# zju3dv/LoG

Hardware: NVIDIA H100
Metric: gaussians_per_s_fwd_bwd (higher is better)
Workload: dtype f32

## Files before the change

### include/log_b200_raster.h

```cpp
#ifndef LOG_B200_RASTER_H
#define LOG_B200_RASTER_H

#include <stdint.h>

#ifdef __cplusplus
extern "C" {
#endif

#define LGR_ABI_VERSION 24
#define LGR_TILE 16

#define LGR_FILTER_ADD 0
#define LGR_FILTER_MAX 1
#define LGR_FILTER_NONE 2

#define LGR_E_BADARG (-1)
#define LGR_E_CAPACITY (-2)
#define LGR_E_UNSUPPORTED (-3)

typedef struct lgr_view {
  int32_t image_height, image_width;
  float tanfovx, tanfovy;
  float scale_modifier;
  int32_t sh_degree;
// ... 15 lines not shown
  uint32_t* contrib_entry_d;
  int32_t* contrib_count_d;
  const int32_t* last_contrib_d;
  const int32_t* region_count_d;
  int64_t region_cap;
  int32_t num_regions;
  int32_t num_channels;
  int32_t log_depth;
  float* splat_ext_d;
  const float* cov3D_precomp_d;
  float* dcov3D_d;
  const float* viewmatrix_d;
  const float* projmatrix_d;
  const float* campos_d;
  const float* bg_d;
} lgr_view;

#define LGR_SPLAT_FLOATS 12
#define LGR_GRAD_FLOATS 12
#define LGR_TILE_SCRATCH_INTS 33
#define LGR_CONTRIB_MAX_LIST (1 << 24)
#define LGR_META_INTS 8

int lgr_abi_version(void);

int lgr_compute_radius(int64_t n, const float* means3D_d, const float* scales_d, const float* rotations_d,
                       const float* projmatrix_d, const float* viewmatrix_d, float focal_x, float focal_y,
                       float tan_fovx, float tan_fovy, float* radii_d, void* stream);

int lgr_mark_visible(int64_t n, const float* means3D_d, const float* viewmatrix_d, uint8_t* visible_d, void* stream);
// ... 207 lines not shown
```

### log_b200/_capi.py

```python
import ctypes
import os

from .build import LIB_PATH

_i32, _i64, _f32, _vp = ctypes.c_int32, ctypes.c_int64, ctypes.c_float, ctypes.c_void_p

LGR_FILTER_ADD, LGR_FILTER_MAX, LGR_FILTER_NONE = 0, 1, 2
LGR_SPLAT_FLOATS = 12
LGR_GRAD_FLOATS = 12
LGR_META_INTS = 8
LGR_TILE_SCRATCH_INTS = 33
LGR_ABI_VERSION = 24
LGR_CONTRIB_MAX_LIST = 1 << 24
LGR_STAGE_HEADER_FLOATS = 64
LGR_ROW_FLOATS = 20

EXPORTS = ('lgr_abi_version', 'lgr_sort_smem_capacity', 'lgr_compute_radius', 'lgr_forward_project',
           'lgr_forward_render', 'lgr_forward_render_device_sized', 'lgr_backward', 'lgr_grad_scatter_add', 'lgr_grad_scatter_add_staged', 'lgr_point_compact', 'lgr_sparse_adam', 'lgr_profile_enable', 'lgr_profile_collect',
           'lgr_profile_kernel_name', 'lgr_shard_send', 'lgr_shard_recv_bin', 'lgr_blend_backward', 'lgr_shard_return_rows',
           'lgr_shard_gather', 'lgr_shard_recv_bin_aux', 'lgr_shard_return_packed', 'lgr_shard_gather_packed', 'lgr_tree_traverse', 'lgr_mark_visible',
           'lgr_ssim_forward', 'lgr_ssim_backward', 'lgr_depth_loss_forward', 'lgr_depth_loss_backward', 'lgr_depth_vis',
           'lgr_counter_update', 'lgr_log_step', 'lgr_prepare_cull', 'lgr_prepare_select')
LGR_SHARD_MAX_RANKS = 32
LGR_PROFILE_KERNELS = 12


class LgrView(ctypes.Structure):
    _fields_ = [('image_height', _i32), ('image_width', _i32), ('tanfovx', _f32), ('tanfovy', _f32),
                ('scale_modifier', _f32), ('sh_degree', _i32), ('sh_coeffs', _i32), ('filter_mode', _i32),
                ('want_aux', _i32), ('tile_row_begin', _i32), ('tile_row_end', _i32),
                ('num_owners', _i32), ('raw_params', _i32), ('band_ids_d', _vp), ('band_blk_d', _vp), ('band_count_d', _vp), ('band_rows_d', _vp), ('band_dsplat_d', _vp), ('tile_rank_d', _vp), ('gather_index_d', _vp), ('pid_map_d', _vp), ('contrib_id_d', _vp), ('contrib_entry_d', _vp), ('contrib_count_d', _vp), ('last_contrib_d', _vp),
                ('region_count_d', _vp), ('region_cap', _i64), ('num_regions', _i32), ('num_channels', _i32), ('log_depth', _i32), ('splat_ext_d', _vp), ('cov3D_precomp_d', _vp), ('dcov3D_d', _vp),
                ('viewmatrix_d', _vp), ('projmatrix_d', _vp), ('campos_d', _vp), ('bg_d', _vp)]


class LgrShardLayout(ctypes.Structure):
    _fields_ = [('num_ranks', _i32), ('my_rank', _i32), ('cap', _i64), ('off_count', _i64), ('off_splat', _i64),
                ('off_radii', _i64), ('off_gid', _i64), ('off_dsplat', _i64), ('off_weight', _i64), ('off_pcount', _i64)]


class LgrTree(ctypes.Structure):
    _fields_ = [('num_points', _i64), ('num_nodes', _i64), ('max_child', _i32), ('max_level', _i32),
                ('node_index_d', _vp), ('tree_d', _vp)]


def tree_scratch_ints(num_points, slots):
    return 8 + 2 * num_points + slots + 2 * ((slots + 255) // 256) + 2 + (slots + 3) // 4

# ... 190 lines not shown
```

### log_b200/csrc/lgr_bin.cu

```cuda
#include "lgr_common.cuh"
#include "lgr_prof.cuh"

namespace lgr {

constexpr int SCAN_THREADS = 1024;
constexpr int SORT_CAP_SMALL_FWD = 4096;

__global__ void __launch_bounds__(SCAN_THREADS)
tile_scan_kernel(int ntiles, int32_t* __restrict__ tile_start ,
                 int32_t* __restrict__ cursor ,
                 int32_t* __restrict__ meta, int small_cap) {
  __shared__ int warp_sum[SCAN_THREADS / 32];
  __shared__ int carry_s, maxl_s, nbig_s;
  const int tid = threadIdx.x, lane = tid & 31, wid = tid >> 5;
  if (tid == 0) { carry_s = 0; maxl_s = 0; nbig_s = 0; }
  __syncthreads();
  int local_max = 0;
  for (int base = 0; base < ntiles; base += SCAN_THREADS) {
    const int i = base + tid;
    const int c = (i < ntiles) ? cursor[i * CSTRIDE] + cursor[i * CSTRIDE + 1] : 0;
    local_max = max(local_max, c);
    int x = c;
#pragma unroll
    for (int o = 1; o < 32; o <<= 1) { const int y = __shfl_up_sync(0xffffffffu, x, o); if (lane >= o) x += y; }
// ... 128 lines not shown
            float4* z = reinterpret_cast<float4*>(v.band_dsplat + (int64_t)id * LGR_GRAD_FLOATS);
            z[0] = z[1] = z[2] = make_float4(0.f, 0.f, 0.f, 0.f);
          }
          i = id;
        }
      }
      int rad = 0;
      float4 r0 = make_float4(0.f, 0.f, 0.f, 0.f), r1 = r0;
      float depth = 0.f;
      if (live) {
        rad = radii[i];
        r0 = ldg4(splat + i * LGR_SPLAT_FLOATS);
        r1 = ldg4(splat + i * LGR_SPLAT_FLOATS + 4);
        depth = __ldg(splat + i * LGR_SPLAT_FLOATS + 11);
        live = rad > 0;
      }
      if (live && v.num_owners == 0 && v.band_dsplat) {
        float4* z = reinterpret_cast<float4*>(v.band_dsplat + i * LGR_GRAD_FLOATS);
        z[0] = z[1] = z[2] = make_float4(0.f, 0.f, 0.f, 0.f);
      }
      int x0 = 0, y0 = 0, x1 = 0, y1 = 0;
      uint32_t key = 0;
      if (live) {
        live = r1.z > 0.f;
        if (live) {
          key = __float_as_uint(depth);
          tile_rect_tight(r0.x, r0.y, rad, r1.z, r1.w, v.gx, v.gy, v.row0, v.row1, x0, y0, x1, y1);
        }
      }
      const int w = x1 - x0, cnt = live ? w * (y1 - y0) : 0;
      const int mine = cnt <= 4 ? cnt : 0;
      int incl = mine;
#pragma unroll
      for (int o = 1; o < 32; o <<= 1) { const int y = __shfl_up_sync(0xffffffffu, incl, o); if (lane >= o) incl += y; }
// ... 445 lines not shown
  LGR_CHECK_LAUNCH();
  return 0;
}

constexpr int LONG_SORT_GRID = 132;

int launch_bin_and_sort(const View& v, int64_t n, int64_t num_inst, int max_len, int num_long, const float* splat,
                        const int32_t* radii, int32_t* tile_start, int32_t* cursor, uint32_t* inst_key,
                        uint32_t* inst_val, uint32_t* inst_tmp, int32_t* sorted_ids, int32_t* meta_dev, cudaStream_t st) {
  if (n == 0) return 0;
  if (meta_dev) {
    const int nt = v.gx * (v.row1 - v.row0);
    clamp_lists_kernel<<<(nt + 256) / 256, 256, 0, st>>>(nt, num_inst, tile_start, meta_dev);
    LGR_CHECK_LAUNCH();
  }
  if (num_inst == 0 && v.num_owners == 0 && v.band_dsplat == nullptr) return 0;
  if (num_inst > 0 && (!inst_tmp || !sorted_ids)) return LGR_E_BADARG;
  const int ntiles = v.gx * (v.row1 - v.row0);
  const int part_smem = part_smem_bytes(v.row1 - v.row0);
  if (part_smem > 160 * 1024) return LGR_E_UNSUPPORTED;
  {
    cudaError_t e = cudaFuncSetAttribute(bin_partition_kernel, cudaFuncAttributeMaxDynamicSharedMemorySize, part_smem);
    if (e != cudaSuccess) return (int)e;
  }
  const int rounds = (int)max((int64_t)1, min((int64_t)PART_ROUNDS, n / ((int64_t)BIN_THREADS * 132 * 16)));
  const int64_t chunk = (int64_t)rounds * BIN_THREADS;
  unsigned blocks = (unsigned)((n + chunk - 1) / chunk);
  if (v.region_count && blocks > (unsigned)LGR_REGION_GRID) blocks = (unsigned)LGR_REGION_GRID;
  unsigned long long* stage = reinterpret_cast<unsigned long long*>(inst_tmp);
  {
    ProfScope ps(K_BIN_SCATTER, st, num_inst > BIN_DIRECT_MAX ? 2 : 1);
// ... 45 lines not shown
```

### log_b200/csrc/lgr_blend.cu

```cuda
#include "lgr_common.cuh"
#include "lgr_prof.cuh"

namespace lgr {

constexpr int BLEND_THREADS = TILE_PIX;
#ifndef LGR_FWD_MIN_CTAS
#define LGR_FWD_MIN_CTAS 5
#endif
#ifndef LGR_BWD_MIN_CTAS
#define LGR_BWD_MIN_CTAS 4
#endif
#ifndef LGR_FWD6_MIN_CTAS
#define LGR_FWD6_MIN_CTAS 4
#endif
#ifndef LGR_BWD6_MIN_CTAS
#define LGR_BWD6_MIN_CTAS 3
#endif
constexpr int BATCH = 256;
constexpr unsigned FULL = 0xffffffffu;

struct SubTile {
  int x, y;
  bool inside;
};
// ... 217 lines not shown
      }
      const int c = __popc(m);
      int incl = c;
#pragma unroll
      for (int d = 1; d < BATCH / 32; d <<= 1) {
        const int y = __shfl_up_sync(FULL, incl, d);
        if (lane >= d) incl += y;
      }
      const unsigned mine = __shfl_sync(FULL, m, warp);
      const int before = __shfl_sync(FULL, incl - c, warp);
      if ((mine >> lane) & 1u) {
        unsigned byte = 0u;
#pragma unroll
        for (int w = 0; w < BLEND_THREADS / 32; w++) byte |= ((s_cb[w * (BATCH / 32) + warp] >> lane) & 1u) << w;
        const int k = beg + n_rec + before + __popc(mine & ((1u << lane) - 1u));
        v.contrib_id[k] = __float_as_int(s_rec[F4 * tid + 2].w);
        v.contrib_entry[k] = byte | ((uint32_t)(base + tid) << 8);
      }
      n_rec += __shfl_sync(FULL, incl, BATCH / 32 - 1);
    }
    base += BATCH;
    if (all_done || base >= len) break;
    cnt = min(BATCH, len - base);
    stage();
  }
  if (REC && tid == 0) v.contrib_count[tile] = n_rec;
  if (st.inside) {
    const int64_t pix = (int64_t)st.y * v.W + st.x, HW = (int64_t)v.H * v.W;
    image[pix] = C0 + T * __ldg(v.bg);
    image[HW + pix] = C1 + T * __ldg(v.bg + 1);
    image[2 * HW + pix] = C2 + T * __ldg(v.bg + 2);
    if (SIX) {
// ... 328 lines not shown
```

### log_b200/csrc/lgr_capi.cu

```cuda
#include "lgr_common.cuh"
#include "lgr_prof.cuh"
#include <math.h>

namespace lgr {
int launch_mark_visible(int64_t, const float*, const float*, uint8_t*, cudaStream_t);
int launch_compute_radius(int64_t, const float*, const float*, const float*, const float*, const float*, float, float,
                          float, float, float*, cudaStream_t);
int launch_project_fwd(const View&, Colour, bool, int64_t, const float*, const float*, const float*, const float*,
                       const float*, const float*, float*, int32_t*, uint8_t*, int32_t*, int32_t*, cudaStream_t);
int launch_project_bwd(const View&, Colour, bool, bool, int64_t, const float*, const float*, const float*, const float*,
                       const float*, const int32_t*, const uint8_t*, const float*, float*, float*, float*, float*, float*,
                       float*, float*, float*, void* const*, int, cudaStream_t);
int launch_grad_scatter_add(int64_t, const float*, int64_t, int64_t, float*, cudaStream_t);
int launch_grad_scatter_add_staged(const float*, int, int64_t, int64_t, int64_t, float*, cudaStream_t);
int launch_band_scan(const View&, cudaStream_t);
int launch_tile_scan(int, int32_t*, int32_t*, int32_t*, bool, cudaStream_t);
int launch_bin_and_sort(const View&, int64_t, int64_t, int, int, const float*, const int32_t*, int32_t*, int32_t*,
                        uint32_t*, uint32_t*, uint32_t*, int32_t*, int32_t*, cudaStream_t);
int sort_smem_capacity();
int launch_blend_fwd(const View&, const int32_t*, const int32_t*, const float*, float*, float*, int32_t*, int32_t*,
                     float*, float*, int32_t*, cudaStream_t);
int launch_sparse_adam(int64_t, int, const int64_t*, const float*, float*, float*, float*, float*, float, float, float, float,
                       float, float, float, cudaStream_t);
int launch_counter_update(const lgr_counter&, int64_t, int64_t, const int64_t*, const int64_t*, const int32_t*, const float*,
// ... 42 lines not shown
  const int lists = (v->contrib_id_d != nullptr) + (v->contrib_entry_d != nullptr) + (v->contrib_count_d != nullptr);
  if (lists != 0 && lists != 3) return false;
  if (v->num_channels != 0 && v->num_channels != 3 && v->num_channels != 6) return false;
  if (v->num_channels == 6 && !v->splat_ext_d) return false;
  if (v->log_depth != 0 && (v->log_depth != 1 || v->num_channels != 6)) return false;
  return true;
}

static int six_channels_check(const lgr_view* v) {
  if (v->num_channels != 6) return 0;
  if (v->num_owners > 0 || v->region_count_d || v->pid_map_d) return LGR_E_UNSUPPORTED;
  if (!v->log_depth && (v->raw_params || v->gather_index_d)) return LGR_E_UNSUPPORTED;
  return 0;
}

static int colour_source(const lgr_view* v, int64_t n, const float* colors_precomp_d, const float* shs_d, Colour* c) {
  const bool six_precomp = v->num_channels == 6 && !v->log_depth;
  if (six_precomp && shs_d) return LGR_E_UNSUPPORTED;
  const bool log_sh = v->raw_params && colors_precomp_d && shs_d;
  if (!log_sh && (colors_precomp_d != nullptr) == (shs_d != nullptr) && n > 0) return LGR_E_BADARG;
  *c = log_sh ? Colour::LOG_SH : shs_d ? Colour::SH : six_precomp ? Colour::RGB6 : Colour::RGB;
  return 0;
}

extern "C" {

int lgr_abi_version(void) { return LGR_ABI_VERSION; }

int32_t lgr_sort_smem_capacity(void) { return sort_smem_capacity(); }

// ... 50 lines not shown
  if (rc) return rc;
  return launch_tile_scan(ntiles, tile_start_d, tile_cursor_d, meta_d, false, st);
}

int lgr_forward_render(const lgr_view* view, int64_t n, int64_t num_instances, int32_t max_tile_len,
                       int32_t num_long_tiles, const float* splat_d, const int32_t* radii_d, const int32_t* tile_start_d,
                       int32_t* tile_cursor_d, uint32_t* inst_key_d, uint32_t* inst_val_d, uint32_t* inst_tmp_d,
                       int32_t* sorted_ids_d, float* image_d, float* final_T_d, int32_t* n_contrib_d,
                       int32_t* point_id_pixel_d, float* point_weight_pixel_d, float* point_weight_d,
                       int32_t* point_count_d, void* stream) {
  if (!view_ok(view) || n < 0 || num_instances < 0 || num_long_tiles < 0 || !tile_start_d || !tile_cursor_d || !image_d || !final_T_d ||
      !n_contrib_d)
    return LGR_E_BADARG;
  if (num_instances > 0 && (!inst_key_d || !inst_val_d || !inst_tmp_d || !sorted_ids_d || !splat_d || !radii_d)) return LGR_E_BADARG;
  if (const int rc6 = six_channels_check(view)) return rc6;
  if (view->want_aux && (!point_id_pixel_d || !point_weight_pixel_d || (n > 0 && !point_weight_d))) return LGR_E_BADARG;
  if (num_instances > 0x7fffffffLL) return LGR_E_UNSUPPORTED;
  if (view->contrib_id_d && max_tile_len > LGR_CONTRIB_MAX_LIST) return LGR_E_UNSUPPORTED;
  cudaStream_t st = (cudaStream_t)stream;
  const View v = make_view(view, n);
  int rc = launch_bin_and_sort(v, n, num_instances, max_tile_len, num_long_tiles, splat_d, radii_d, const_cast<int32_t*>(tile_start_d), tile_cursor_d,
                               inst_key_d, inst_val_d, inst_tmp_d, sorted_ids_d, nullptr, st);
  if (rc) return rc;
  return launch_blend_fwd(v, tile_start_d, sorted_ids_d, splat_d, image_d, final_T_d, n_contrib_d, point_id_pixel_d,
                          point_weight_pixel_d, point_weight_d, view->want_aux ? point_count_d : nullptr, st);
}

int lgr_forward_render_device_sized(const lgr_view* view, int64_t n, int64_t instance_capacity, int32_t* meta_d,
                                    const float* splat_d, const int32_t* radii_d, int32_t* tile_start_d,
                                    int32_t* tile_cursor_d, uint32_t* inst_key_d, uint32_t* inst_val_d,
                                    uint32_t* inst_tmp_d, int32_t* sorted_ids_d, float* image_d, float* final_T_d, int32_t* n_contrib_d,
                                    int32_t* point_id_pixel_d, float* point_weight_pixel_d, float* point_weight_d,
                                    int32_t* point_count_d, void* stream) {
  if (!view_ok(view) || n < 0 || instance_capacity <= 0 || !meta_d || !tile_start_d || !tile_cursor_d || !image_d || !final_T_d ||
      !n_contrib_d || !inst_key_d || !inst_val_d || !inst_tmp_d || !sorted_ids_d)
    return LGR_E_BADARG;
  if (n > 0 && (!splat_d || !radii_d)) return LGR_E_BADARG;
  if (const int rc6 = six_channels_check(view)) return rc6;
  if (view->want_aux && (!point_id_pixel_d || !point_weight_pixel_d || (n > 0 && !point_weight_d))) return LGR_E_BADARG;
  if (instance_capacity > 0x7fffffffLL) return LGR_E_UNSUPPORTED;
  cudaStream_t st = (cudaStream_t)stream;
  const View v = make_view(view, n);
  int rc = launch_bin_and_sort(v, n, instance_capacity, 0, 0, splat_d, radii_d, tile_start_d, tile_cursor_d, inst_key_d, inst_val_d,
                               inst_tmp_d, sorted_ids_d, meta_d, st);
  if (rc) return rc;
  return launch_blend_fwd(v, tile_start_d, sorted_ids_d, splat_d, image_d, final_T_d, n_contrib_d, point_id_pixel_d,
                          point_weight_pixel_d, point_weight_d, view->want_aux ? point_count_d : nullptr, st);
}

int lgr_backward(const lgr_view* view, int64_t n, int64_t num_instances, const float* means3D_d,
                 const float* opacities_d, const float* scales_d, const float* rotations_d,
                 const float* colors_precomp_d, const float* shs_d, const float* splat_d, const int32_t* radii_d,
                 const uint8_t* clamped_d, const int32_t* tile_start_d, const int32_t* sorted_ids_d,
                 const float* image_d, const float* dL_dimage_d, float* dsplat_d,
                 float* dmeans3D_d, float* dmeans2D_d, float* dopacities_d, float* dscales_d, float* drotations_d,
                 float* dcolors_d, float* dshs_d, float* grad_rows_d, void* const* peer_stage_d, int32_t my_rank,
                 int64_t num_rows, void* stream) {
  if (!view_ok(view) || n < 0 || !tile_start_d || !image_d || !dL_dimage_d) return LGR_E_BADARG;
  if (const int rc6 = six_channels_check(view)) return rc6;
  const bool rows_mode = grad_rows_d || peer_stage_d;
  if (view->num_channels == 6 && rows_mode) return LGR_E_UNSUPPORTED;
  Colour c;
  if (const int rc = colour_source(view, n, colors_precomp_d, shs_d, &c)) return rc;
  if (n == 0) return 0;
  if (c == Colour::LOG_SH && (!dshs_d || !view->campos_d || view->num_owners > 0)) return LGR_E_BADARG;
  const bool cov3d = view->cov3D_precomp_d != nullptr;
  if (!means3D_d || (!cov3d && (!scales_d || !rotations_d)) || !splat_d || !radii_d || !dsplat_d) return LGR_E_BADARG;
  if (cov3d && (!view->dcov3D_d || view->raw_params || view->num_owners > 0 || grad_rows_d || peer_stage_d)) return LGR_E_BADARG;
  if (view->raw_params && (!opacities_d || c == Colour::SH)) return LGR_E_BADARG;
  if (rows_mode) {
    if (view->num_owners <= 0 || c == Colour::SH) return LGR_E_BADARG;
    if (peer_stage_d && (my_rank < 0 || my_rank >= view->num_owners)) return LGR_E_BADARG;
    if (num_rows < 0 || num_rows > n) return LGR_E_BADARG;
  } else {
// ... 344 lines not shown
```

### log_b200/csrc/lgr_common.cuh

```cuda
#pragma once
#include <cuda_runtime.h>
#include <stdint.h>

#include "../../include/log_b200_raster.h"

namespace lgr {

constexpr int TILE = LGR_TILE;
constexpr int TILE_PIX = TILE * TILE;
constexpr float NEAR_Z = 0.2f;
constexpr float ALPHA_MAX = 0.99f;
constexpr float ALPHA_MIN = 1.0f / 255.0f;
constexpr float T_STOP = 1e-4f;
constexpr float FILTER_VAR = 0.3f;
constexpr float CLAMP_FOV = 1.3f;
constexpr int CSTRIDE = 32;
constexpr float LOG2E = 1.4426950408889634f;
constexpr float LN2 = 0.6931471805599453f;

enum class Colour { RGB, SH, LOG_SH, RGB6 };

struct View {
  int H, W, gx, gy;
  int row0, row1;
  float tanfovx, tanfovy, fx, fy, scale_mod;
  int sh_degree, sh_K, filter_mode, want_aux;
  int raw_params;
  int num_owners, owner_chunk;
  int32_t* band_ids;
  int32_t* band_blk;
  int32_t* band_count;
  int32_t* band_rows;
  float* band_dsplat;
  const int64_t* gather;
  const int32_t* pid_map;
  int32_t* contrib_id;
  uint32_t* contrib_entry;
  int32_t* contrib_count;
  const int32_t* last_contrib;
  const int32_t* region_count;
  int64_t region_cap;
  int regions;
  const float* cov3d;
  float* dcov3d;
  int band_blocks;
  const float* view;
  const float* proj;
  const float* campos;
  const float* bg;
  int num_channels;
  int log_depth;
  float* splat_ext;
};

inline View make_view(const lgr_view* v, int64_t n = 0) {
  View o;
  o.num_owners = v->num_owners; o.band_ids = v->band_ids_d; o.band_blk = v->band_blk_d; o.band_count = v->band_count_d; o.band_rows = v->band_rows_d; o.band_dsplat = v->band_dsplat_d; o.gather = v->gather_index_d; o.pid_map = v->pid_map_d; o.contrib_id = v->contrib_id_d; o.contrib_entry = v->contrib_entry_d; o.contrib_count = v->contrib_count_d; o.last_contrib = v->last_contrib_d;
  o.region_count = v->region_count_d; o.region_cap = v->region_cap; o.regions = v->region_count_d ? v->num_regions : 0;
  o.cov3d = v->cov3D_precomp_d; o.dcov3d = v->dcov3D_d;
  o.owner_chunk = o.num_owners > 0 ? (int)LGR_OWNER_CHUNK(n, (int64_t)o.num_owners) : 256;
  if (o.owner_chunk < 256) o.owner_chunk = 256;
  o.band_blocks = (int)((n + 255) / 256);
  o.H = v->image_height; o.W = v->image_width;
  o.gx = (o.W + TILE - 1) / TILE; o.gy = (o.H + TILE - 1) / TILE;
  o.row0 = v->tile_row_begin; o.row1 = v->tile_row_end;
  if (o.row0 == 0 && o.row1 == 0) o.row1 = o.gy;
  o.tanfovx = v->tanfovx; o.tanfovy = v->tanfovy;
  o.fx = o.W / (2.0f * v->tanfovx); o.fy = o.H / (2.0f * v->tanfovy);
  o.scale_mod = v->scale_modifier;
  o.sh_degree = v->sh_degree; o.sh_K = v->sh_coeffs; o.filter_mode = v->filter_mode; o.want_aux = v->want_aux;
  o.raw_params = v->raw_params;
  o.view = v->viewmatrix_d; o.proj = v->projmatrix_d; o.campos = v->campos_d; o.bg = v->bg_d;
// ... 213 lines not shown
```

### log_b200/csrc/lgr_project.cu

```cuda
#include "lgr_common.cuh"
#include "lgr_prof.cuh"

namespace lgr {

constexpr int PROJ_THREADS = 256;

__device__ __forceinline__ void load3(const float* __restrict__ p, int64_t i, float o[3]) {
  o[0] = __ldg(p + 3 * i); o[1] = __ldg(p + 3 * i + 1); o[2] = __ldg(p + 3 * i + 2);
}

__device__ __forceinline__ void load_cov3d(const float* cov, int64_t i, float Sg[9]) {
  const float* c6 = cov + 6 * i;
  const float cxx = __ldg(c6), cxy = __ldg(c6 + 1), cxz = __ldg(c6 + 2), cyy = __ldg(c6 + 3), cyz = __ldg(c6 + 4), czz = __ldg(c6 + 5);
  Sg[0] = cxx; Sg[1] = cxy; Sg[2] = cxz; Sg[3] = cxy; Sg[4] = cyy; Sg[5] = cyz; Sg[6] = cxz; Sg[7] = cyz; Sg[8] = czz;
}

__device__ __forceinline__ void sh_dir_basis(const float p[3], const float* cam, int deg, float B[16]) {
  const float d[3] = {p[0] - cam[0], p[1] - cam[1], p[2] - cam[2]};
  const float inv = 1.0f / sqrtf(d[0] * d[0] + d[1] * d[1] + d[2] * d[2]);
  sh_basis(deg, d[0] * inv, d[1] * inv, d[2] * inv, B);
}

__device__ __forceinline__ void sh_accumulate(const float* sh, const float B[16], int first, int nb, float rgb[3]) {
  for (int k = first; k < nb; k++) {
// ... 257 lines not shown
    int64_t first = 0;
    for (int o = 0; o <= my_rank && o < v.num_owners - 1; o++) first += v.band_count[o];
    if (my_rank == v.num_owners - 1) first = 0;
    blk = (blk + first / PROJ_THREADS) % gridDim.x;
  }
  int64_t i = blk * PROJ_THREADS + threadIdx.x;
  const bool active = i < n;
  if (!ROWS && !active) return;
  int64_t row = 0;
  if (ROWS && active) {
    row = i;
    i = v.band_rows[row];
  }
  float dm[3] = {0.f, 0.f, 0.f}, dm2[2] = {0.f, 0.f}, dop = 0.f, dsc[3] = {0.f, 0.f, 0.f}, dq[4] = {0.f, 0.f, 0.f, 0.f};
  float drgb[3] = {0.f, 0.f, 0.f}, dext[3] = {0.f, 0.f, 0.f};
  const bool live = active && radii[i] > 0;
  const int64_t src = (v.gather && live) ? v.gather[i] : i;
  const int K = v.sh_K;
  if (live) {
    const float4 g0 = ldg4(dsplat + i * LGR_GRAD_FLOATS);
    const float4 g1 = ldg4(dsplat + i * LGR_GRAD_FLOATS + 4);
    const float4 g2 = ldg4(dsplat + i * LGR_GRAD_FLOATS + 8);
    float p[3], s0[3], s[3], R[9], Sg[9];
    load3(means, src, p);
    float4 q = make_float4(1.f, 0.f, 0.f, 0.f);
    float q_inv = 1.0f;
    if (COV3D) {
      load_cov3d(v.cov3d, src, Sg);
    } else {
      load3(scales, src, s0);
      q = ldg4(rots + 4 * src);
// ... 391 lines not shown
```

### log_b200/gathered.py

```python
from types import SimpleNamespace
from typing import Dict, Optional

import torch

from ._capi import LGR_FILTER_MAX, LGR_FILTER_NONE
from .rasterizer import rasterize_backward, rasterize_forward


class GatheredParams(dict):

    def __init__(self, keys):
        super().__init__({k: SimpleNamespace(grad=None) for k in keys})


class _RenderGathered(torch.autograd.Function):
    @staticmethod
    def forward(ctx, means2D, settings, tables, index, sh_degree_tables, filter_mode, params, log_depth=False):
        colors, shs = tables['colors'], tables.get('shs')
        use_shs = shs is not None and settings.sh_degree > 0
        out = rasterize_forward(settings, tables['xyz'], tables['opacity'].reshape(-1), tables['scaling'], tables['rotation'],
                                colors, shs if use_shs else None, filter_mode, True, raw_params=True, gather_index=index,
                                log_depth=log_depth)
        image, radii, pid, pwp, pw, state = out
        state.image = None
        ctx.state, ctx.tables, ctx.params, ctx.use_shs = state, tables, params, use_shs
        ctx.save_for_backward(image)
        ctx.mark_non_differentiable(radii, pid, pwp, pw, state.point_count)
        return image, radii, pid, pwp, pw, state.point_count

    @staticmethod
    def backward(ctx, grad_image, *unused):
        (image,) = ctx.saved_tensors
        t = ctx.tables
        ctx.state.image = image
        dm3, dm2, dop, dsc, drot, dcol, dsh = rasterize_backward(ctx.state, grad_image, t['xyz'], t['opacity'].reshape(-1), t['scaling'],
                                                                 t['rotation'], t['colors'], t.get('shs') if ctx.use_shs else None)
        ctx.state.image = None
        p = ctx.params
        p['xyz'].grad, p['scaling'].grad, p['rotation'].grad = dm3, dsc, drot
        p['opacity'].grad, p['colors'].grad = dop.reshape(-1, 1), dcol
        if 'shs' in p:
            p['shs'].grad = dsh
        return dm2, None, None, None, None, None, None, None


def render_gathered(settings, tables: Dict[str, torch.Tensor], index: torch.Tensor, means2D: torch.Tensor, use_filter: bool = True,
                    params: Optional[GatheredParams] = None, render_depth: bool = False):
    if params is None:
        params = GatheredParams([k for k in ('xyz', 'scaling', 'rotation', 'opacity', 'colors', 'shs') if k in tables])
    tabs = {k: v.detach() for k, v in tables.items()}
    out = _RenderGathered.apply(means2D, settings, tabs, index, None, LGR_FILTER_MAX if use_filter else LGR_FILTER_NONE, params,
                                bool(render_depth))
    return out[:5], out[5], params
```

### log_b200/rasterizer.py

```python
import ctypes
from typing import NamedTuple, Optional

import torch
import torch.nn as nn

from . import _capi
from ._capi import LGR_FILTER_ADD, LGR_FILTER_MAX, LGR_FILTER_NONE, LgrView

PREZERO_DSPLAT = bool(int(__import__('os').environ.get('LGR_PREZERO_DSPLAT', '0')))
CONTRIB_BITS = bool(int(__import__('os').environ.get('LGR_CONTRIB_BITS', '1')))
FLAVOUR_STOCK = 'stock'
FLAVOUR_FORK = 'fork'


class GaussianRasterizationSettings(NamedTuple):
    image_height: int
    image_width: int
    tanfovx: float
    tanfovy: float
    bg: torch.Tensor
    scale_modifier: float
    viewmatrix: torch.Tensor
    projmatrix: torch.Tensor
    sh_degree: int
# ... 92 lines not shown
        if used:
            raise _capi.LgrError(f'six colour channels (colors_precomp (N,6)) are not available with {what}')
    if settings.bg.numel() != 6:
        raise _capi.LgrError(f'six colour channels need a background of 6 entries (raster_settings.bg), got {settings.bg.numel()}')
    return 6


def use_contrib_lists(D, max_tile_len):
    return CONTRIB_BITS and D > 0 and (max_tile_len is None or max_tile_len <= _capi.LGR_CONTRIB_MAX_LIST)


class RasterState:
    __slots__ = ('view', 'keep', 'n', 'num_instances', 'max_tile_len', 'stock_instances', 'num_visible', 'splat',
                 'radii', 'clamped', 'tile_start', 'sorted_ids', 'final_T', 'n_contrib', 'image', 'sh', 'num_owners',
                 'band_ids', 'band_count', 'band_counts_host', 'point_count', 'meta', 'cov3D', 'dcov3D', 'contrib',
                 'channels', 'splat_ext', 'log_depth')

    def read_stats(self):
        m = self.meta.tolist()
        return dict(num_instances=int(m[0]), max_tile_len=int(m[1]), stock_instances=(m[2] & 0xffffffff) | ((m[3] & 0xffffffff) << 32),
                    num_visible=int(m[4]), overflow=int(m[6]))

    def contrib_lists(self):
        if self.contrib is None:
            return None
        D = self.num_instances
        return self.contrib[:D], self.contrib[D:2 * D], self.contrib[2 * D:]


def rasterize_forward(settings, means3D, opacities, scales, rotations, colors_precomp, shs, filter_mode, want_aux,
                      tile_rows=None, num_owners=0, raw_params=False, prezero_dsplat=None, gather_index=None,
# ... 9 lines not shown
    for name, t in (('opacities', opacities), ('scales', scales), ('rotations', rotations), ('colors_precomp', colors_precomp),
                    ('shs', shs), ('cov3D_precomp', cov3D_precomp), ('viewmatrix', settings.viewmatrix), ('projmatrix', settings.projmatrix), ('bg', settings.bg)):
        if t is not None and t.device != dev:
            raise _capi.LgrError(f'{name} is on {t.device}, means3D on {dev}: all inputs of a call must share one device')
    n = int(means3D.shape[0])
    keep = []
    if gather_index is not None:
        if gather_index.dtype != torch.int64 or gather_index.device != dev or gather_index.dim() != 1:
            raise _capi.LgrError('gather_index must be a 1-D int64 tensor on the inputs\' device')
        if num_owners > 0:
            raise _capi.LgrError('gather_index is not available in band mode')
        gather_index = gather_index.contiguous()
        keep.append(gather_index)
        n = int(gather_index.shape[0])
    K = 0 if shs is None else int(shs.shape[1])
    band_ids = band_count = band_blk = band_rows = band_dsplat = None
    if prezero_dsplat is None:
        prezero_dsplat = PREZERO_DSPLAT and torch.is_grad_enabled()
    if num_owners == 0 and prezero_dsplat:
        band_dsplat = torch.empty((max(n, 1), _capi.LGR_GRAD_FLOATS), dtype=torch.float32, device=dev)
    if num_owners > 0:
        band_rows = torch.empty((max(n, 1),), dtype=torch.int32, device=dev)
        band_dsplat = torch.empty((max(n, 1), _capi.LGR_GRAD_FLOATS), dtype=torch.float32, device=dev)
        nb = (n + 255) // 256
        band_ids = torch.empty((max(256 * nb, 1),), dtype=torch.int32, device=dev)
        band_blk = torch.empty((2 * nb + 1,), dtype=torch.int32, device=dev)
        band_count = torch.empty((num_owners,), dtype=torch.int32, device=dev)
    splat_ext = torch.empty((max(n, 1), 4), dtype=torch.float32, device=dev) if channels == 6 else None
    keep.append(splat_ext)
    view = _make_view(settings, filter_mode, want_aux, K, tile_rows, keep, num_owners, band_ids, band_count, band_blk, band_rows, band_dsplat,
                      raw_params, gather_index, cov3D_precomp=cov3D_precomp, splat_ext=splat_ext, log_depth=log_depth)
    H, W = view.image_height, view.image_width
    gx, gy = (W + 15) // 16, (H + 15) // 16
    rows = gy if tile_rows is None else int(tile_rows[1]) - int(tile_rows[0])
    ntiles = gx * rows
# ... 18 lines not shown
    if want_aux:
        pc = torch.zeros((n,), **i32)
        pid = torch.empty((H, W), **i32) if tile_rows is None else torch.full((H, W), -1, **i32)
        pwp = torch.empty((H, W), **f32) if tile_rows is None else torch.zeros((H, W), **f32)
        pw = torch.zeros((n,), **f32)
    if instance_capacity:
        if num_owners > 0:
            raise _capi.LgrError('instance_capacity (device-sized call) is not available in band mode')
        D, max_len, num_long, stock_D, m = int(instance_capacity), None, None, None, None
        inst_key, inst_val = torch.empty((D,), **u32), torch.empty((D,), **u32)
        inst_tmp = torch.empty((2 * D,), **u32)
        sorted_ids = torch.empty((D,), **i32)
        contrib = torch.empty((2 * D + ntiles,), **i32) if use_contrib_lists(D, None) else None
        keep.append(contrib)
        set_contrib_lists(view, contrib, D, n_contrib)
        _capi.check(lib.lgr_forward_render_device_sized(ctypes.byref(view), n, D, _ptr(meta), _ptr(splat), _ptr(radii), _ptr(tile_start),
                                                        _ptr(tile_cursor), _ptr(inst_key), _ptr(inst_val), _ptr(inst_tmp), _ptr(sorted_ids), _ptr(image),
                                                        _ptr(final_T), _ptr(n_contrib), _ptr(pid), _ptr(pwp), _ptr(pw), _ptr(pc), st),
                    'lgr_forward_render_device_sized')
    else:
        m = (meta if band_count is None else torch.cat([meta, band_count])).tolist()
        D, max_len, num_long = int(m[0]), int(m[1]), int(m[5])
        stock_D = (m[2] & 0xffffffff) | ((m[3] & 0xffffffff) << 32)
        if D < 0 or stock_D > 0x7fffffff:
            raise _capi.LgrError(f'this view needs {stock_D} (Gaussian, tile) instances by the stock rule (D = {m[0] & 0xffffffff} binned, '
                                 f'{m[4]} of {n} Gaussians visible, longest tile list {max_len}): more than 2^31 - 1 is unsupported')
        inst_key = torch.empty((D,), **u32)
        inst_val = torch.empty((D,), **u32)
        inst_tmp = torch.empty((2 * D,), **u32)
        sorted_ids = torch.empty((D,), **i32)
        contrib = torch.empty((2 * D + ntiles,), **i32) if use_contrib_lists(D, max_len) else None
        keep.append(contrib)
        set_contrib_lists(view, contrib, D, n_contrib)
        _capi.check(lib.lgr_forward_render(ctypes.byref(view), n, D, max_len, num_long, _ptr(splat), _ptr(radii), _ptr(tile_start),
                                           _ptr(tile_cursor), _ptr(inst_key), _ptr(inst_val), _ptr(inst_tmp),
                                           _ptr(sorted_ids), _ptr(image), _ptr(final_T), _ptr(n_contrib), _ptr(pid),
                                           _ptr(pwp), _ptr(pw), _ptr(pc), st), 'lgr_forward_render')
    s = RasterState()
    s.view, s.keep, s.n, s.num_instances, s.max_tile_len = view, keep, n, D, max_len
    s.stock_instances, s.num_visible = stock_D, (int(m[4]) if m is not None else None)
    s.meta = meta
    s.cov3D, s.dcov3D = cov3D_precomp, None
    s.splat, s.radii, s.clamped, s.tile_start, s.sorted_ids = splat, radii, clamped, tile_start, sorted_ids
    s.final_T, s.n_contrib, s.image, s.sh = final_T, n_contrib, image, shs is not None
    s.point_count = pc
    s.contrib = contrib
    s.channels, s.splat_ext, s.log_depth = channels, splat_ext, bool(log_depth)
    s.num_owners, s.band_ids, s.band_count = num_owners, (band_ids, band_blk, band_rows, band_dsplat), band_count
    s.band_counts_host = [int(x) for x in m[_capi.LGR_META_INTS:]] if num_owners > 0 else None
    return image, radii, pid, pwp, pw, s


def rasterize_backward(state: RasterState, grad_image, means3D, opacities, scales, rotations, colors_precomp, shs,
                       peer_stage=None, my_rank=0):
    lib = _capi.load()
    dev = means3D.device
    n = state.n
    f32 = dict(dtype=torch.float32, device=dev)
    g = _f32c(grad_image, 'grad_image', dev)
    if state.band_ids[3] is not None:
        dsplat = state.band_ids[3]
        state.band_ids = state.band_ids[:3] + (None,)
    else:
        dsplat = torch.zeros((n, _capi.LGR_GRAD_FLOATS), **f32)
    if state.num_owners > 0:
        m_rows = sum(state.band_counts_host)
        if peer_stage is not None:
            _capi.check(lib.lgr_backward(ctypes.byref(state.view), n, state.num_instances, _ptr(means3D), _ptr(opacities),
                                         _ptr(scales), _ptr(rotations), _ptr(colors_precomp), None, _ptr(state.splat),
                                         _ptr(state.radii), None, _ptr(state.tile_start), _ptr(state.sorted_ids),
                                         _ptr(state.image), _ptr(g), _ptr(dsplat), None, None, None, None, None, None, None,
                                         None, ctypes.c_void_p(peer_stage.data_ptr()), int(my_rank), m_rows, _stream(dev)), 'lgr_backward')
            return None
        rows = torch.empty((m_rows, _capi.LGR_ROW_FLOATS), **f32)
        _capi.check(lib.lgr_backward(ctypes.byref(state.view), n, state.num_instances, _ptr(means3D), _ptr(opacities),
                                     _ptr(scales), _ptr(rotations), _ptr(colors_precomp), None, _ptr(state.splat),
                                     _ptr(state.radii), None, _ptr(state.tile_start), _ptr(state.sorted_ids),
                                     _ptr(state.image), _ptr(g), _ptr(dsplat), None, None, None, None, None, None, None,
                                     ctypes.c_void_p(rows.data_ptr()) if rows.numel() else _ptr(dsplat), None, 0, m_rows, _stream(dev)),
# ... 119 lines not shown
        if cov3D_precomp is not None and raw_params:
            raise NotImplementedError('raw_params (LoG\'s fused activations) needs scales and rotations, not cov3D_precomp')
        fork = self.flavour == FLAVOUR_FORK
        if fork:
            filter_mode = LGR_FILTER_MAX if use_filter else LGR_FILTER_NONE
        else:
            filter_mode = LGR_FILTER_ADD
        if raw_params and shs is not None and colors_precomp is None:
            raise NotImplementedError('raw_params with SH: pass the raw DC colours as colors_precomp and the REST coefficients '
                                      '(LoG layout, activation.py:27-34) as shs')
        needs_grad = torch.is_grad_enabled() and any(t is not None and t.requires_grad for t in
                                                     (means3D, means2D, opacities, colors_precomp, shs, scales, rotations, cov3D_precomp))
        holder = {}
        out = _RasterizeGaussians.apply(means3D, means2D, opacities, colors_precomp, shs, scales, rotations,
                                        self.raster_settings, filter_mode, fork, self.tile_rows, raw_params,
                                        PREZERO_DSPLAT and needs_grad, self.instance_capacity, holder, cov3D_precomp,
                                        bool(render_depth))
        self.last_state = holder.get('state')
        if self.raster_settings.debug and means3D.is_cuda:
            torch.cuda.synchronize(means3D.device)
        self.last_point_count = out[5] if fork else None
        return out[:5] if fork else out


class StockGaussianRasterizer(GaussianRasterizer):
    flavour = FLAVOUR_STOCK


def compute_radius(means3D, scales, rotations, projmatrix, viewmatrix, focal_x, focal_y, tan_fovx, tan_fovy):
    lib = _capi.load()
    m = _f32c(means3D, 'means3D')
# ... 9 lines not shown
```

Baseline: 1.841 billion.

## Zero gradient rows only for composited gaussians via blend-time bitmask

Instead of zero-filling the whole dsplat buffer (or every visible gaussian's row) before backward, the blend kernel sets a per-gaussian bit with atomicOr when it records a contribution, and the first recorder zeroes that gaussian's gradient row. The backward projection then treats only composited gaussians as live, skipping gradient work for visible but non-contributing ones. Prezeroing is now on by default whenever grad is enabled. This removes a full-size memset and per-gaussian projection-backward work, at the cost of atomics in the blend record loop and a new bitmask buffer.

```diff
diff --git a/include/log_b200_raster.h b/include/log_b200_raster.h
--- a/include/log_b200_raster.h
+++ b/include/log_b200_raster.h
@@ -7,7 +7,7 @@
 extern "C" {
 #endif
 
-#define LGR_ABI_VERSION 24
+#define LGR_ABI_VERSION 25
 #define LGR_TILE 16
 
 #define LGR_FILTER_ADD 0
@@ -53,6 +53,7 @@
   const float* projmatrix_d;
   const float* campos_d;
   const float* bg_d;
+  uint32_t* composited_d;
 } lgr_view;
 
 #define LGR_SPLAT_FLOATS 12
diff --git a/log_b200/_capi.py b/log_b200/_capi.py
--- a/log_b200/_capi.py
+++ b/log_b200/_capi.py
@@ -10,7 +10,7 @@
 LGR_GRAD_FLOATS = 12
 LGR_META_INTS = 8
 LGR_TILE_SCRATCH_INTS = 33
-LGR_ABI_VERSION = 24
+LGR_ABI_VERSION = 25
 LGR_CONTRIB_MAX_LIST = 1 << 24
 LGR_STAGE_HEADER_FLOATS = 64
 LGR_ROW_FLOATS = 20
@@ -31,7 +31,7 @@
                 ('want_aux', _i32), ('tile_row_begin', _i32), ('tile_row_end', _i32),
                 ('num_owners', _i32), ('raw_params', _i32), ('band_ids_d', _vp), ('band_blk_d', _vp), ('band_count_d', _vp), ('band_rows_d', _vp), ('band_dsplat_d', _vp), ('tile_rank_d', _vp), ('gather_index_d', _vp), ('pid_map_d', _vp), ('contrib_id_d', _vp), ('contrib_entry_d', _vp), ('contrib_count_d', _vp), ('last_contrib_d', _vp),
                 ('region_count_d', _vp), ('region_cap', _i64), ('num_regions', _i32), ('num_channels', _i32), ('log_depth', _i32), ('splat_ext_d', _vp), ('cov3D_precomp_d', _vp), ('dcov3D_d', _vp),
-                ('viewmatrix_d', _vp), ('projmatrix_d', _vp), ('campos_d', _vp), ('bg_d', _vp)]
+                ('viewmatrix_d', _vp), ('projmatrix_d', _vp), ('campos_d', _vp), ('bg_d', _vp), ('composited_d', _vp)]
 
 
 class LgrShardLayout(ctypes.Structure):
diff --git a/log_b200/csrc/lgr_bin.cu b/log_b200/csrc/lgr_bin.cu
--- a/log_b200/csrc/lgr_bin.cu
+++ b/log_b200/csrc/lgr_bin.cu
@@ -166,10 +166,6 @@
         r1 = ldg4(splat + i * LGR_SPLAT_FLOATS + 4);
         depth = __ldg(splat + i * LGR_SPLAT_FLOATS + 11);
         live = rad > 0;
-      }
-      if (live && v.num_owners == 0 && v.band_dsplat) {
-        float4* z = reinterpret_cast<float4*>(v.band_dsplat + i * LGR_GRAD_FLOATS);
-        z[0] = z[1] = z[2] = make_float4(0.f, 0.f, 0.f, 0.f);
       }
       int x0 = 0, y0 = 0, x1 = 0, y1 = 0;
       uint32_t key = 0;
@@ -645,7 +641,7 @@
     clamp_lists_kernel<<<(nt + 256) / 256, 256, 0, st>>>(nt, num_inst, tile_start, meta_dev);
     LGR_CHECK_LAUNCH();
   }
-  if (num_inst == 0 && v.num_owners == 0 && v.band_dsplat == nullptr) return 0;
+  if (num_inst == 0 && v.num_owners == 0) return 0;
   if (num_inst > 0 && (!inst_tmp || !sorted_ids)) return LGR_E_BADARG;
   const int ntiles = v.gx * (v.row1 - v.row0);
   const int part_smem = part_smem_bytes(v.row1 - v.row0);
diff --git a/log_b200/csrc/lgr_blend.cu b/log_b200/csrc/lgr_blend.cu
--- a/log_b200/csrc/lgr_blend.cu
+++ b/log_b200/csrc/lgr_blend.cu
@@ -255,8 +255,16 @@
 #pragma unroll
         for (int w = 0; w < BLEND_THREADS / 32; w++) byte |= ((s_cb[w * (BATCH / 32) + warp] >> lane) & 1u) << w;
         const int k = beg + n_rec + before + __popc(mine & ((1u << lane) - 1u));
-        v.contrib_id[k] = __float_as_int(s_rec[F4 * tid + 2].w);
+        const int id = __float_as_int(s_rec[F4 * tid + 2].w);
+        v.contrib_id[k] = id;
         v.contrib_entry[k] = byte | ((uint32_t)(base + tid) << 8);
+        if (v.composited) {
+          const unsigned bit = 1u << (id & 31);
+          if (!(atomicOr(v.composited + (id >> 5), bit) & bit)) {
+            float4* z = reinterpret_cast<float4*>(v.band_dsplat + (int64_t)id * LGR_GRAD_FLOATS);
+            z[0] = z[1] = z[2] = make_float4(0.f, 0.f, 0.f, 0.f);
+          }
+        }
       }
       n_rec += __shfl_sync(FULL, incl, BATCH / 32 - 1);
     }
diff --git a/log_b200/csrc/lgr_capi.cu b/log_b200/csrc/lgr_capi.cu
--- a/log_b200/csrc/lgr_capi.cu
+++ b/log_b200/csrc/lgr_capi.cu
@@ -80,6 +80,13 @@
   return 0;
 }
 
+static int composited_check(const lgr_view* v) {
+  if (!v->composited_d) return 0;
+  if (!v->band_dsplat_d || v->num_owners != 0 || v->region_count_d || v->pid_map_d) return LGR_E_UNSUPPORTED;
+  if (!v->contrib_id_d) return LGR_E_BADARG;
+  return 0;
+}
+
 static int colour_source(const lgr_view* v, int64_t n, const float* colors_precomp_d, const float* shs_d, Colour* c) {
   const bool six_precomp = v->num_channels == 6 && !v->log_depth;
   if (six_precomp && shs_d) return LGR_E_UNSUPPORTED;
@@ -160,6 +167,7 @@
     return LGR_E_BADARG;
   if (num_instances > 0 && (!inst_key_d || !inst_val_d || !inst_tmp_d || !sorted_ids_d || !splat_d || !radii_d)) return LGR_E_BADARG;
   if (const int rc6 = six_channels_check(view)) return rc6;
+  if (const int rcc = composited_check(view)) return rcc;
   if (view->want_aux && (!point_id_pixel_d || !point_weight_pixel_d || (n > 0 && !point_weight_d))) return LGR_E_BADARG;
   if (num_instances > 0x7fffffffLL) return LGR_E_UNSUPPORTED;
   if (view->contrib_id_d && max_tile_len > LGR_CONTRIB_MAX_LIST) return LGR_E_UNSUPPORTED;
@@ -183,6 +191,7 @@
     return LGR_E_BADARG;
   if (n > 0 && (!splat_d || !radii_d)) return LGR_E_BADARG;
   if (const int rc6 = six_channels_check(view)) return rc6;
+  if (const int rcc = composited_check(view)) return rcc;
   if (view->want_aux && (!point_id_pixel_d || !point_weight_pixel_d || (n > 0 && !point_weight_d))) return LGR_E_BADARG;
   if (instance_capacity > 0x7fffffffLL) return LGR_E_UNSUPPORTED;
   cudaStream_t st = (cudaStream_t)stream;
@@ -204,6 +213,7 @@
                  int64_t num_rows, void* stream) {
   if (!view_ok(view) || n < 0 || !tile_start_d || !image_d || !dL_dimage_d) return LGR_E_BADARG;
   if (const int rc6 = six_channels_check(view)) return rc6;
+  if (const int rcc = composited_check(view)) return rcc;
   const bool rows_mode = grad_rows_d || peer_stage_d;
   if (view->num_channels == 6 && rows_mode) return LGR_E_UNSUPPORTED;
   Colour c;
diff --git a/log_b200/csrc/lgr_common.cuh b/log_b200/csrc/lgr_common.cuh
--- a/log_b200/csrc/lgr_common.cuh
+++ b/log_b200/csrc/lgr_common.cuh
@@ -32,6 +32,7 @@
   int32_t* band_count;
   int32_t* band_rows;
   float* band_dsplat;
+  uint32_t* composited;
   const int64_t* gather;
   const int32_t* pid_map;
   int32_t* contrib_id;
@@ -55,7 +56,7 @@
 
 inline View make_view(const lgr_view* v, int64_t n = 0) {
   View o;
-  o.num_owners = v->num_owners; o.band_ids = v->band_ids_d; o.band_blk = v->band_blk_d; o.band_count = v->band_count_d; o.band_rows = v->band_rows_d; o.band_dsplat = v->band_dsplat_d; o.gather = v->gather_index_d; o.pid_map = v->pid_map_d; o.contrib_id = v->contrib_id_d; o.contrib_entry = v->contrib_entry_d; o.contrib_count = v->contrib_count_d; o.last_contrib = v->last_contrib_d;
+  o.num_owners = v->num_owners; o.band_ids = v->band_ids_d; o.band_blk = v->band_blk_d; o.band_count = v->band_count_d; o.band_rows = v->band_rows_d; o.band_dsplat = v->band_dsplat_d; o.composited = v->composited_d; o.gather = v->gather_index_d; o.pid_map = v->pid_map_d; o.contrib_id = v->contrib_id_d; o.contrib_entry = v->contrib_entry_d; o.contrib_count = v->contrib_count_d; o.last_contrib = v->last_contrib_d;
   o.region_count = v->region_count_d; o.region_cap = v->region_cap; o.regions = v->region_count_d ? v->num_regions : 0;
   o.cov3d = v->cov3D_precomp_d; o.dcov3d = v->dcov3D_d;
   o.owner_chunk = o.num_owners > 0 ? (int)LGR_OWNER_CHUNK(n, (int64_t)o.num_owners) : 256;
diff --git a/log_b200/csrc/lgr_project.cu b/log_b200/csrc/lgr_project.cu
--- a/log_b200/csrc/lgr_project.cu
+++ b/log_b200/csrc/lgr_project.cu
@@ -295,7 +295,7 @@
   }
   float dm[3] = {0.f, 0.f, 0.f}, dm2[2] = {0.f, 0.f}, dop = 0.f, dsc[3] = {0.f, 0.f, 0.f}, dq[4] = {0.f, 0.f, 0.f, 0.f};
   float drgb[3] = {0.f, 0.f, 0.f}, dext[3] = {0.f, 0.f, 0.f};
-  const bool live = active && radii[i] > 0;
+  const bool live = active && (v.composited ? (v.composited[i >> 5] >> (i & 31)) & 1u : radii[i] > 0);
   const int64_t src = (v.gather && live) ? v.gather[i] : i;
   const int K = v.sh_K;
   if (live) {
diff --git a/log_b200/gathered.py b/log_b200/gathered.py
--- a/log_b200/gathered.py
+++ b/log_b200/gathered.py
@@ -15,12 +15,12 @@
 
 class _RenderGathered(torch.autograd.Function):
     @staticmethod
-    def forward(ctx, means2D, settings, tables, index, sh_degree_tables, filter_mode, params, log_depth=False):
+    def forward(ctx, means2D, settings, tables, index, sh_degree_tables, filter_mode, params, log_depth=False, needs_grad=False):
         colors, shs = tables['colors'], tables.get('shs')
         use_shs = shs is not None and settings.sh_degree > 0
         out = rasterize_forward(settings, tables['xyz'], tables['opacity'].reshape(-1), tables['scaling'], tables['rotation'],
                                 colors, shs if use_shs else None, filter_mode, True, raw_params=True, gather_index=index,
-                                log_depth=log_depth)
+                                log_depth=log_depth, prezero_dsplat=needs_grad)
         image, radii, pid, pwp, pw, state = out
         state.image = None
         ctx.state, ctx.tables, ctx.params, ctx.use_shs = state, tables, params, use_shs
@@ -41,7 +41,7 @@
         p['opacity'].grad, p['colors'].grad = dop.reshape(-1, 1), dcol
         if 'shs' in p:
             p['shs'].grad = dsh
-        return dm2, None, None, None, None, None, None, None
+        return dm2, None, None, None, None, None, None, None, None
 
 
 def render_gathered(settings, tables: Dict[str, torch.Tensor], index: torch.Tensor, means2D: torch.Tensor, use_filter: bool = True,
@@ -49,6 +49,7 @@
     if params is None:
         params = GatheredParams([k for k in ('xyz', 'scaling', 'rotation', 'opacity', 'colors', 'shs') if k in tables])
     tabs = {k: v.detach() for k, v in tables.items()}
+    needs_grad = torch.is_grad_enabled() and means2D.requires_grad
     out = _RenderGathered.apply(means2D, settings, tabs, index, None, LGR_FILTER_MAX if use_filter else LGR_FILTER_NONE, params,
-                                bool(render_depth))
+                                bool(render_depth), needs_grad)
     return out[:5], out[5], params
diff --git a/log_b200/rasterizer.py b/log_b200/rasterizer.py
--- a/log_b200/rasterizer.py
+++ b/log_b200/rasterizer.py
@@ -7,7 +7,6 @@
 from . import _capi
 from ._capi import LGR_FILTER_ADD, LGR_FILTER_MAX, LGR_FILTER_NONE, LgrView
 
-PREZERO_DSPLAT = bool(int(__import__('os').environ.get('LGR_PREZERO_DSPLAT', '0')))
 CONTRIB_BITS = bool(int(__import__('os').environ.get('LGR_CONTRIB_BITS', '1')))
 FLAVOUR_STOCK = 'stock'
 FLAVOUR_FORK = 'fork'
@@ -130,7 +129,7 @@
     __slots__ = ('view', 'keep', 'n', 'num_instances', 'max_tile_len', 'stock_instances', 'num_visible', 'splat',
                  'radii', 'clamped', 'tile_start', 'sorted_ids', 'final_T', 'n_contrib', 'image', 'sh', 'num_owners',
                  'band_ids', 'band_count', 'band_counts_host', 'point_count', 'meta', 'cov3D', 'dcov3D', 'contrib',
-                 'channels', 'splat_ext', 'log_depth')
+                 'channels', 'splat_ext', 'log_depth', 'composited')
 
     def read_stats(self):
         m = self.meta.tolist()
@@ -170,11 +169,9 @@
         keep.append(gather_index)
         n = int(gather_index.shape[0])
     K = 0 if shs is None else int(shs.shape[1])
-    band_ids = band_count = band_blk = band_rows = band_dsplat = None
+    band_ids = band_count = band_blk = band_rows = band_dsplat = composited = None
     if prezero_dsplat is None:
-        prezero_dsplat = PREZERO_DSPLAT and torch.is_grad_enabled()
-    if num_owners == 0 and prezero_dsplat:
-        band_dsplat = torch.empty((max(n, 1), _capi.LGR_GRAD_FLOATS), dtype=torch.float32, device=dev)
+        prezero_dsplat = torch.is_grad_enabled()
     if num_owners > 0:
         band_rows = torch.empty((max(n, 1),), dtype=torch.int32, device=dev)
         band_dsplat = torch.empty((max(n, 1), _capi.LGR_GRAD_FLOATS), dtype=torch.float32, device=dev)
@@ -223,6 +220,7 @@
         contrib = torch.empty((2 * D + ntiles,), **i32) if use_contrib_lists(D, None) else None
         keep.append(contrib)
         set_contrib_lists(view, contrib, D, n_contrib)
+        band_dsplat, composited = _composited_rows(view, n, contrib, num_owners, prezero_dsplat, band_dsplat, keep)
         _capi.check(lib.lgr_forward_render_device_sized(ctypes.byref(view), n, D, _ptr(meta), _ptr(splat), _ptr(radii), _ptr(tile_start),
                                                         _ptr(tile_cursor), _ptr(inst_key), _ptr(inst_val), _ptr(inst_tmp), _ptr(sorted_ids), _ptr(image),
                                                         _ptr(final_T), _ptr(n_contrib), _ptr(pid), _ptr(pwp), _ptr(pw), _ptr(pc), st),
@@ -241,6 +239,7 @@
         contrib = torch.empty((2 * D + ntiles,), **i32) if use_contrib_lists(D, max_len) else None
         keep.append(contrib)
         set_contrib_lists(view, contrib, D, n_contrib)
+        band_dsplat, composited = _composited_rows(view, n, contrib, num_owners, prezero_dsplat, band_dsplat, keep)
         _capi.check(lib.lgr_forward_render(ctypes.byref(view), n, D, max_len, num_long, _ptr(splat), _ptr(radii), _ptr(tile_start),
                                            _ptr(tile_cursor), _ptr(inst_key), _ptr(inst_val), _ptr(inst_tmp),
                                            _ptr(sorted_ids), _ptr(image), _ptr(final_T), _ptr(n_contrib), _ptr(pid),
@@ -255,9 +254,21 @@
     s.point_count = pc
     s.contrib = contrib
     s.channels, s.splat_ext, s.log_depth = channels, splat_ext, bool(log_depth)
+    s.composited = composited
     s.num_owners, s.band_ids, s.band_count = num_owners, (band_ids, band_blk, band_rows, band_dsplat), band_count
     s.band_counts_host = [int(x) for x in m[_capi.LGR_META_INTS:]] if num_owners > 0 else None
     return image, radii, pid, pwp, pw, s
+
+
+def _composited_rows(view, n, contrib, num_owners, backward_follows, band_dsplat, keep):
+    if num_owners > 0 or not backward_follows or contrib is None:
+        return band_dsplat, None
+    dev = contrib.device
+    band_dsplat = torch.empty((max(n, 1), _capi.LGR_GRAD_FLOATS), dtype=torch.float32, device=dev)
+    composited = torch.zeros(((n + 31) // 32,), dtype=torch.int32, device=dev)
+    keep.append(composited)
+    view.band_dsplat_d, view.composited_d = band_dsplat.data_ptr(), composited.data_ptr()
+    return band_dsplat, composited
 
 
 def rasterize_backward(state: RasterState, grad_image, means3D, opacities, scales, rotations, colors_precomp, shs,
@@ -272,6 +283,7 @@
         state.band_ids = state.band_ids[:3] + (None,)
     else:
         dsplat = torch.zeros((n, _capi.LGR_GRAD_FLOATS), **f32)
+        state.view.composited_d = None
     if state.num_owners > 0:
         m_rows = sum(state.band_counts_host)
         if peer_stage is not None:
@@ -421,7 +433,7 @@
         holder = {}
         out = _RasterizeGaussians.apply(means3D, means2D, opacities, colors_precomp, shs, scales, rotations,
                                         self.raster_settings, filter_mode, fork, self.tile_rows, raw_params,
-                                        PREZERO_DSPLAT and needs_grad, self.instance_capacity, holder, cov3D_precomp,
+                                        needs_grad, self.instance_capacity, holder, cov3D_precomp,
                                         bool(render_depth))
         self.last_state = holder.get('state')
         if self.raster_settings.debug and means3D.is_cuda:
```

Measured after the change: 1.887 billion, median of 6. +2.5%, better.
